# ath92/splat-renderer

Hardware: AMD Instinct MI355X
Metric: Msplats/sec (higher is better)
Workload: dtype f32

## Files before the change

### include/splat.h

```cpp
#ifndef SPLAT_H
#define SPLAT_H

#include <stddef.h>
#include <stdint.h>

#ifdef __cplusplus
extern "C" {
#endif

#define SPLAT_ABI_VERSION 3

#define SPLAT_OK 0
#define SPLAT_ERR_INVALID (-1)
#define SPLAT_ERR_HIP (-2)
#define SPLAT_ERR_OOM (-3)
#define SPLAT_ERR_CAPACITY (-4)
#define SPLAT_ERR_STATE (-5)
#define SPLAT_ERR_NO_DEVICE (-6)
#define SPLAT_ERR_COMM (-7)
#define SPLAT_ERR_RETRY (-8)

typedef struct splat_ctx splat_ctx;
typedef struct splat_sorter splat_sorter;
typedef struct splat_binner splat_binner;
// ... 46 lines not shown
                  uint32_t pr_stride_vec4, uint32_t n, void *projected, void *keys, void *payload,
                  uint32_t n_padded);

int splat_extract_keys(splat_ctx *ctx, const void *projected, uint32_t n, uint32_t n_padded,
                       void *keys, void *payload);

int splat_sort_create(splat_ctx *ctx, uint32_t capacity, splat_sorter **out);
void splat_sort_destroy(splat_sorter *s);
uint32_t splat_sort_capacity(const splat_sorter *s);
void *splat_sort_keys(splat_sorter *s);
void *splat_sort_payload(splat_sorter *s);
int splat_sort_run(splat_sorter *s, uint32_t n, uint32_t bit_begin, uint32_t bit_end);
void *splat_sort_sorted_payload(splat_sorter *s);
void *splat_sort_sorted_keys(splat_sorter *s);
int splat_probe_lds_atomic_order(splat_ctx *ctx, uint64_t *mismatches);
int splat_sort_set_mode(splat_sorter *s, int mode);
int splat_rank_status(splat_ctx *ctx, int *policy, int *atomics_ordered, uint32_t *order_faults);
#ifdef SPLAT_TEST_HOOKS
int splat_debug_inject_order_fault(splat_ctx *ctx, uint32_t tile, uint32_t position);
int splat_debug_set_tile_order(splat_ctx *ctx, const void *order_dptr);
int splat_debug_set_tile_sort_order(splat_ctx *ctx, const void *order_dptr);
int splat_debug_rerun_tile_sort(splat_ctx *ctx, splat_binner *binner);
int splat_debug_tile_sort_launches(splat_ctx *ctx, uint32_t *launches);
int splat_debug_lds_rate(splat_ctx *ctx, int kind, uint32_t workgroups_per_cu, uint32_t iters, float *ms);
#endif
int splat_composite_forget_history(splat_ctx *ctx);
int splat_composite_options(splat_ctx *ctx, int kernel, int ahead, int predict);

int splat_scan_u32(splat_ctx *ctx, const void *in, void *out, uint32_t n, void *total_dptr);

int splat_bin_create(splat_ctx *ctx, uint32_t tile_size, splat_binner **out);
void splat_bin_destroy(splat_binner *b);
int splat_bin_run(splat_binner *b, const void *projected, uint32_t n_splats, const void *sorted,
                  uint32_t n_sorted, uint32_t width, uint32_t height, uint32_t tile_row0,
                  uint32_t tile_row1);
uint32_t splat_bin_tile_size(const splat_binner *b);
int splat_bin_counts(splat_binner *b, void **dptr);
int splat_bin_offsets(splat_binner *b, void **dptr);
int splat_bin_indices(splat_binner *b, void **dptr);
int splat_bin_total(splat_binner *b, uint64_t *total_pairs);
#define SPLAT_FRAME_ORDER_DEFAULT (-1)
#define SPLAT_FRAME_SORT_FIRST 0
#define SPLAT_FRAME_TILE_FIRST 1
int splat_bin_set_frame_order(splat_binner *b, int order);
int splat_bin_dims(splat_binner *b, uint32_t *ntx, uint32_t *nty);

// ... 229 lines not shown
```

### splat_renderer_amd/_lib.py

```python
import ctypes as C
import os

_HERE = os.path.dirname(os.path.abspath(__file__))
LIB_PATH = os.environ.get("SPLAT_LIB_PATH") or os.path.join(_HERE, "libsplat_hip.so")

OK = 0
ERR_NAMES = {-1: "INVALID", -2: "HIP", -3: "OOM", -4: "CAPACITY", -5: "STATE", -6: "NO_DEVICE", -7: "COMM", -8: "RETRY"}
ERR_CAPACITY, ERR_RETRY = -4, -8
RENDER_AGAIN = (ERR_CAPACITY, ERR_RETRY)

STAGE_PROJECT, STAGE_SORT, STAGE_BIN, STAGE_COMPOSITE, STAGE_EXCHANGE, STAGE_BIN_SCATTER, STAGE_BIN_PASS2, STAGE_BIN_TILE_SORT = range(8)
STAGE_NAMES = ("project", "sort", "bin", "composite", "exchange", "bin_scatter", "bin_second_pass", "bin_tile_sort")
TIMING_COUNT_ENTRIES = 0x80000000
MODE_FRONT_TO_BACK, MODE_REFERENCE_LITERAL = 0, 1
RECORDS_PROJECTED, RECORDS_COMPACT, RECORDS_DISC48, RECORDS_LIT32 = 0, 1, 2, 3
FOOTPRINT_ISOTROPIC, FOOTPRINT_DISC, FOOTPRINT_ELLIPSOID = 0, 1, 2
U32_MAX = 0xFFFFFFFF


class SplatError(RuntimeError):
    def __init__(self, code, msg):
        super().__init__(f"libsplat_hip error {ERR_NAMES.get(code, code)}: {msg}")
        self.code = code

# ... 140 lines not shown
    "splat_band_keys": (_i, [_vp, _vp, _vp, _u32, _u32, _u32, _u32, _u32, _u32, C.POINTER(_u32)]),
    "splat_sdf_gradients": (_i, [_vp, _vp, _u32, _vp, _u32, _vp]),
    "splat_sdf_update_positions": (_i, [_vp, _vp, _vp, _u32, _vp]),
    "splat_sdf_scale_factors": (_i, [_vp, _vp, _u32, _vp, _u32, _vp]),
    "splat_sdf_curvature": (_i, [_vp, _vp, _vp, _u32, _vp]),
    "splat_sdf_seed_positions": (_i, [_vp, C.POINTER(C.c_float), C.POINTER(C.c_float), _u32, C.c_uint64, _vp]),
    "splat_sdf_generate": (_i, [_vp, _vp, _u32, C.POINTER(C.c_float), C.POINTER(C.c_float), C.c_uint64, _vp, _u32, _u32, _vp, _vp, _vp, _vp]),
    "splat_point_frame": (_i, [_vp, _vp, C.POINTER(C.c_float), _vp, _u32, _vp, _u32, _vp, _u32, _u32, _u32, _u32, _vp, _vp, _vp, _vp]),
    "splat_comm_unique_id": (_i, [_vp]),
    "splat_comm_init": (_i, [_vp, _i, _i, _vp, _pvp]),
    "splat_comm_destroy": (None, [_vp]),
    "splat_comm_rank": (_i, [_vp, C.POINTER(_i), C.POINTER(_i)]),
    "splat_comm_count": (_i, [_vp, C.POINTER(_i), C.POINTER(_i)]),
    "splat_allgather_records": (_i, [_vp, _vp, _vp, _vp, _sz]),
}
COMM_ID_BYTES = 128
HOOK_SIGNATURES = {
    "splat_debug_inject_order_fault": (_i, [_vp, _u32, _u32]),
    "splat_debug_set_tile_order": (_i, [_vp, _vp]),
    "splat_debug_set_tile_sort_order": (_i, [_vp, _vp]),
    "splat_debug_rerun_tile_sort": (_i, [_vp, _vp]),
    "splat_debug_tile_sort_launches": (_i, [_vp, C.POINTER(_u32)]),
    "splat_debug_lds_rate": (_i, [_vp, _i, _u32, _u32, C.POINTER(C.c_float)]),
}
HOOKS_LIB_PATH = os.path.join(_HERE, "libsplat_hip_hooks.so")

_lib = None


class _Bound:

    def __getattr__(self, name):
        if name in HOOK_SIGNATURES:
            raise AttributeError(f"libsplat_hip: {name} is a test hook: the shipped library does not carry it; run with "
                                 f"SPLAT_LIB_PATH={HOOKS_LIB_PATH} (the -DSPLAT_TEST_HOOKS build)")
        raise AttributeError(f"libsplat_hip: {name} is not declared in splat_renderer_amd._lib.SIGNATURES")


def load():
    global _lib
    if _lib is not None:
        return _lib
    if not os.path.exists(LIB_PATH):
        raise ImportError(
            f"{LIB_PATH} not found: build it with `python -c 'import __graft_entry__ as g; g.build()'` "
            "(hipcc --offload-arch=gfx950). splat_renderer_amd has no CPU fallback.")
# ... 25 lines not shown
```

### splat_renderer_amd/csrc/common.h

```cpp
#pragma once

#include <hip/hip_runtime.h>
#include <stdint.h>
#include <string>

#include "../../include/splat.h"

constexpr int kWave = 64;

#include <vector>
struct StageTimer {
    std::vector<hipEvent_t> beg, end;
    size_t used = 0;
    uint32_t tick = 0;
};
struct PxHistory {
    uint64_t key = 0;
    uint32_t *mem = nullptr;
    uint32_t cap = 0, parity = 0, streak = 0;
    uint64_t last_use = 0;
};
constexpr int PX_HISTORIES = 4;

struct splat_ctx {
    int device = 0;
    hipStream_t stream = nullptr;
    bool own_stream = false;
    std::string err;
    bool timing = false;
    int lds_atomic_ordered = -1;
    int rank_policy = 0;
    uint32_t order_faults = 0;
#ifdef SPLAT_TEST_HOOKS
    const uint32_t *debug_tile_order = nullptr;
    const uint32_t *debug_sort_order = nullptr;
    uint32_t inject_order_fault = 0;
    uint32_t inject_order_position = 0;
    uint32_t tile_sort_launches = 0;
#endif
    int opt_composite_kernel = -1, opt_px_ahead = 0, opt_px_predict = -1;
    PxHistory px_hist[PX_HISTORIES];
    uint64_t px_clock = 0;
    uint32_t timing_mask = 0xffffffffu;
    uint32_t timing_every = 1;
    StageTimer timers[SPLAT_STAGE_COUNT];
    void *scan_ws = nullptr;
    size_t scan_ws_bytes = 0;
    unsigned long long *d_consumed = nullptr;
    uint32_t consumed_tiles = 0;
    uint2 *d_window_counts = nullptr;
    uint32_t window_counts_cap = 0;
    void *pinned = nullptr;
    size_t pinned_bytes = 0;
};

int ctx_fail(splat_ctx *ctx, int code, const char *what, hipError_t e = hipSuccess);
bool composite_uses_px(const splat_ctx *ctx, uint32_t ntx, uint32_t nty);

int ctx_ensure_scan_ws(splat_ctx *ctx, size_t bytes);
int ctx_ensure_pinned(splat_ctx *ctx, size_t bytes);
int ctx_ensure_consumed(splat_ctx *ctx, uint32_t tiles);
// ... 193 lines not shown
```

### splat_renderer_amd/csrc/context.hip

```cpp
#include "common.h"

#include <cstdio>
#include <cstring>

static thread_local std::string g_tls_err = "";

int ctx_fail(splat_ctx *ctx, int code, const char *what, hipError_t e) {
    char buf[512];
    if (e != hipSuccess)
        snprintf(buf, sizeof buf, "%s: %s (%d)", what, hipGetErrorString(e), (int)e);
    else
        snprintf(buf, sizeof buf, "%s", what);
    if (ctx) ctx->err = buf;
    g_tls_err = buf;
    return code;
}

int ctx_ensure_scan_ws(splat_ctx *ctx, size_t bytes) {
    if (ctx->scan_ws_bytes >= bytes) return SPLAT_OK;
    if (ctx->scan_ws) {
        HIP_TRY(ctx, hipStreamSynchronize(ctx->stream));
        HIP_TRY(ctx, hipFree(ctx->scan_ws));
        ctx->scan_ws = nullptr;
        ctx->scan_ws_bytes = 0;
// ... 55 lines not shown
    (void)hipEventRecord(t.end[t.used], ctx->stream);
    ++t.used;
}

static int ctx_create_impl(int device, void *stream, bool have_stream, splat_ctx **out) {
    if (!out) return ctx_fail(nullptr, SPLAT_ERR_INVALID, "splat_ctx_create: out is NULL");
    *out = nullptr;
    int count = 0;
    hipError_t e = hipGetDeviceCount(&count);
    if (e != hipSuccess || count <= 0)
        return ctx_fail(nullptr, SPLAT_ERR_NO_DEVICE, "no HIP device visible (this library has no CPU fallback)", e);
    if (device < 0 || device >= count) return ctx_fail(nullptr, SPLAT_ERR_INVALID, "device ordinal out of range");
    e = hipSetDevice(device);
    if (e != hipSuccess) return ctx_fail(nullptr, SPLAT_ERR_HIP, "hipSetDevice", e);
    hipDeviceProp_t prop;
    e = hipGetDeviceProperties(&prop, device);
    if (e != hipSuccess) return ctx_fail(nullptr, SPLAT_ERR_HIP, "hipGetDeviceProperties", e);
    if (strncmp(prop.gcnArchName, "gfx950", 6) != 0) {
        std::string m = std::string("device is ") + prop.gcnArchName + "; libsplat_hip is built for gfx950 (MI355X) only";
        return ctx_fail(nullptr, SPLAT_ERR_NO_DEVICE, m.c_str());
    }
    splat_ctx *ctx = new splat_ctx();
    ctx->device = device;
    if (have_stream) {
        ctx->stream = (hipStream_t)stream;
        ctx->own_stream = false;
    } else {
        e = hipStreamCreateWithFlags(&ctx->stream, hipStreamNonBlocking);
        if (e != hipSuccess) {
            delete ctx;
            return ctx_fail(nullptr, SPLAT_ERR_HIP, "hipStreamCreate", e);
        }
        ctx->own_stream = true;
    }
    *out = ctx;
    return SPLAT_OK;
}

extern "C" {

int splat_abi_version(void) { return SPLAT_ABI_VERSION; }

int splat_ctx_create(int device_ordinal, splat_ctx **out) { return ctx_create_impl(device_ordinal, nullptr, false, out); }

int splat_ctx_create_on_stream(int device_ordinal, void *hip_stream, splat_ctx **out) {
    return ctx_create_impl(device_ordinal, hip_stream, true, out);
// ... 171 lines not shown
```

### splat_renderer_amd/csrc/frame.hip

```cpp
#include "common.h"
#include "tile_range.h"
#include "disc.h"
#include "ellipsoid.h"
#include "shade.h"

#include <cstdlib>

__device__ __forceinline__ uint32_t depth_key_of(float depth) {
    uint32_t bits = __float_as_uint(depth);
    uint32_t mask = ((bits >> 31) == 1u) ? 0xffffffffu : 0x80000000u;
    return bits ^ mask;
}

__global__ __launch_bounds__(256) void k_band_flag(const float4 *__restrict__ projected, uint32_t n, uint32_t width,
                                                   uint32_t height, uint32_t tile, uint32_t ntx, uint32_t nty, uint32_t row0,
                                                   uint32_t row1, uint32_t *__restrict__ flags) {
    uint32_t i = blockIdx.x * 256u + threadIdx.x;
    if (i >= n) return;
    uint32_t a, b, c, d;
    flags[i] = tile_range(projected[(size_t)i * 2], width, height, tile, ntx, nty, row0, row1, a, b, c, d) ? 1u : 0u;
}

__global__ __launch_bounds__(256) void k_band_scatter(const float4 *__restrict__ projected, uint32_t n,
                                                      const uint32_t *__restrict__ slot, const uint32_t *__restrict__ total,
// ... 645 lines not shown
                                                "in all)");
    int rc = SPLAT_OK;
    uint32_t *range32 = nullptr;
    uint2 *range_wide = nullptr;
    const BinParams bp = {width, height, tile, ntx, nty, row0, row1, (row0 > 0 || row1 < nty) ? 1u : 0u};
    if (ell && bp.skip_outside)
        return ctx_fail(ctx, SPLAT_ERR_INVALID, "splat_render_frame_ellipsoids: the ellipsoid footprint has no band frame (render every tile row)");
    if (fast) {
        rc = binner_reserve_range32(binner, n);
        if (rc != SPLAT_OK) return rc;
        range32 = binner->range32;
    } else if (wide) {
        rc = binner_reserve_range_wide(binner, n);
        if (rc != SPLAT_OK) return rc;
        range_wide = reinterpret_cast<uint2 *>(binner->range32);
    }
    ARG_CHECK(ctx, (((uintptr_t)props | (uintptr_t)projected) & 15) == 0);
    const bool tile_first = fast && frame_order(binner) == SPLAT_FRAME_TILE_FIRST;
    TfHistOut ho = {};
    const bool band_compact = tile_first && bp.skip_outside && band_compacting(row0, row1, nty);
    if (tile_first) {
        rc = binner_reserve(binner, ntx * nty, n);
        if (rc != SPLAT_OK) return rc;
        const uint32_t block = band_compact ? BTC_GROUP : (n <= TF_SMALL_FRAME_SPLATS && !bp.skip_outside) ? TF_BLOCK_SMALL : TF_BLOCK_LARGE;
        ho = {binner->tf_hist, binner->blocksums, binner->d_total + 1, (1u << tile_id_low_bits(ntx * nty)) - 1u, div_up(n, block), block};
        binner->tf_block = block;
        if (band_compact) {
            rc = binner_reserve_band_idx(ctx, binner, n);
            if (rc != SPLAT_OK) return rc;
            ho.cidx = binner->band_idx;
            ho.kept_groups = sorter->hist;
        }
    }
    if (disc && n > binner->discs_cap) {
        HIP_TRY(ctx, hipStreamSynchronize(ctx->stream));
        if (binner->discs) (void)hipFree(binner->discs);
        binner->discs = nullptr;
        binner->discs_cap = 0;
        if (hipMalloc(&binner->discs, (size_t)n * 48 + 256) != hipSuccess) return ctx_fail(ctx, SPLAT_ERR_OOM, "disc records hipMalloc");
        binner->discs_cap = n;
    }
    if (ctx->timing) {
        rc = ctx_ensure_consumed(ctx, ntx * nty);
        if (rc != SPLAT_OK) return rc;
    }
    const LitIO lio = {(const float4 *)color, (const float4 *)normals, color_stride, 1u, cfg->prelit,
                       lit ? (float4 *)projected : disc_lit ? (float4 *)binner->discs : nullptr};
// ... 87 lines not shown
```

### splat_renderer_amd/csrc/radix_sort.hip

```cpp
#include "common.h"

#include <cstdlib>

constexpr uint32_t RS_THREADS = 256;
constexpr uint32_t RS_ITEMS = RADIX_PART / RS_THREADS;
constexpr uint32_t RS_WAVES = RS_THREADS / 64;

constexpr uint32_t RS_PART_KEYS = RS_ITEMS * RS_THREADS;

__device__ __forceinline__ uint32_t sort_count(uint32_t n_host, const uint32_t *n_dev) {
    if (!n_dev) return n_host;
    const uint32_t v = *n_dev;
    return v < n_host ? v : n_host;
}

__device__ __forceinline__ void hist_add4(uint32_t *h, uint4 v, uint32_t shift, uint32_t mask) {
    const uint32_t a = (v.x >> shift) & mask, b = (v.y >> shift) & mask, c = (v.z >> shift) & mask, d = (v.w >> shift) & mask;
    if (a == b && b == c && c == d) {
        atomicAdd(&h[a], 4u);
    } else {
        atomicAdd(&h[a], 1u);
        atomicAdd(&h[b], 1u);
        atomicAdd(&h[c], 1u);
        atomicAdd(&h[d], 1u);
// ... 580 lines not shown
    if (!ctx) return ctx_fail(nullptr, SPLAT_ERR_INVALID, "ctx is NULL");
    ctx->debug_sort_order = (const uint32_t *)order_dptr;
    return SPLAT_OK;
}

int splat_debug_set_tile_order(splat_ctx *ctx, const void *order_dptr) {
    if (!ctx) return ctx_fail(nullptr, SPLAT_ERR_INVALID, "ctx is NULL");
    ctx->debug_tile_order = (const uint32_t *)order_dptr;
    return SPLAT_OK;
}

int splat_debug_lds_rate(splat_ctx *ctx, int kind, uint32_t workgroups_per_cu, uint32_t iters, float *ms) {
    if (!ctx || !ms) return ctx_fail(ctx, SPLAT_ERR_INVALID, "ctx/ms is NULL");
    ARG_CHECK(ctx, kind >= 0 && kind <= 2 && workgroups_per_cu >= 1 && workgroups_per_cu <= 8 && iters >= 1 && iters <= (1u << 20));
    return radix_probe_lds_rate(ctx, kind, workgroups_per_cu, iters, ms);
}

int splat_debug_tile_sort_launches(splat_ctx *ctx, uint32_t *launches) {
    if (!ctx || !launches) return ctx_fail(nullptr, SPLAT_ERR_INVALID, "ctx/launches is NULL");
    *launches = ctx->tile_sort_launches;
    return SPLAT_OK;
}

int splat_debug_inject_order_fault(splat_ctx *ctx, uint32_t tile, uint32_t position) {
    if (!ctx) return ctx_fail(nullptr, SPLAT_ERR_INVALID, "ctx is NULL");
    ARG_CHECK(ctx, tile != 0xffffffffu);
    ARG_CHECK(ctx, position < 0x3fffffffu);
    ctx->inject_order_fault = tile + 1u;
    ctx->inject_order_position = position;
    return SPLAT_OK;
}
#endif

int splat_probe_lds_atomic_order(splat_ctx *ctx, uint64_t *mismatches) {
    if (!ctx || !mismatches) return ctx_fail(nullptr, SPLAT_ERR_INVALID, "ctx/mismatches is NULL");
    return radix_probe_lds_atomic_order(ctx, mismatches);
}

void *splat_sort_sorted_keys(splat_sorter *s) {
    if (!s) return nullptr;
    return s->result_in_primary ? s->keys : s->keys_b;
}

}
```

### splat_renderer_amd/csrc/tile_first.hip

```cpp
#include "common.h"
#include "tile_range.h"

constexpr uint32_t TF_THREADS = 256;
constexpr uint32_t TF_STAGE = 4096;
static_assert(TF_BLOCK_LARGE == 1024 && TF_BLOCK_SMALL == 256, "the stage word packs the block-local slot in 10 bits; blocks are 256 x {4, 1}");

__device__ __forceinline__ uint32_t range32_hits(uint32_t r) {
    const uint32_t tx0 = r & 0xffu, tx1 = (r >> 8) & 0xffu, ty0 = (r >> 16) & 0xffu, ty1 = r >> 24;
    return (tx0 > tx1 || ty0 > ty1) ? 0u : (tx1 - tx0 + 1) * (ty1 - ty0 + 1);
}

constexpr uint32_t TS_THREADS = 256, TS_WAVES = 4;
constexpr uint32_t TS_LONG_ITEMS = 24;
constexpr uint32_t TS_LDS_ELEMS = 5888;
constexpr uint32_t TS_CHUNK_ITEMS = 16;

struct TileSortShared {
    uint32_t wave_hist[TS_WAVES][256];
    uint32_t digit_base[256];
    uint32_t wave_sums[TS_WAVES];
    uint32_t kmin, kmax;
};

template <bool RANK_ATOMIC>
// ... 32 lines not shown
        const uint32_t t = __shfl_up(incl, s);
        if ((int)lane >= s) incl += t;
    }
    if (lane == 63) wave_sums[w] = incl;
    __syncthreads();
    const uint32_t wprefix = (w > 0 ? wave_sums[0] : 0u) + (w > 1 ? wave_sums[1] : 0u) + (w > 2 ? wave_sums[2] : 0u);
    __syncthreads();
    return wprefix + incl - v;
}

constexpr uint32_t TFS_ITEMS = TF_STAGE / TF_THREADS;

struct TfScatterShared {
    uint32_t wave_hist[TS_WAVES][256];
    uint32_t digit_base[256];
    uint32_t global_base[256];
    uint32_t wave_sums[TS_WAVES];
};

#ifndef TF_SCATTER_WAVES
#define TF_SCATTER_WAVES 5
#endif
constexpr uint32_t TF_GROUP = 4096;
template <bool RANK_ATOMIC, uint32_t TF_PER_THREAD, bool COMPACTED = false>
__global__ __launch_bounds__(TF_THREADS, TF_SCATTER_WAVES) void k_tf_scatter(const uint32_t *__restrict__ range32,
                                                           const uint32_t *__restrict__ depth_keys, uint32_t n, uint32_t ntx,
                                                           uint32_t mask, uint32_t num_parts,
                                                           const uint32_t *__restrict__ scanned_hist,
                                                           const uint32_t *__restrict__ totals, uint32_t *__restrict__ d_total,
                                                           uint32_t pair_limit, uint32_t *__restrict__ overflow,
                                                           uint8_t *__restrict__ out_hi, uint2 *__restrict__ out_val,
                                                           uint32_t lo_bits, uint32_t align_m1, TfRuns runs,
                                                           uint32_t *__restrict__ offsets_out, uint32_t tiles, uint32_t *report,
                                                           uint32_t seq, const uint32_t *__restrict__ cidx,
                                                           const uint32_t *__restrict__ kept, uint32_t xcd_per) {
    static_assert(!COMPACTED || TF_PER_THREAD == 4, "compacted groups are read four splats per thread");
    const uint32_t blk = xcd_block_of(blockIdx.x, xcd_per);
    if (blk >= num_parts) return;
    __shared__ TfScatterShared sh;
    __shared__ uint32_t wsum[4];
    __shared__ uint32_t stage[TF_STAGE];
    __shared__ uint32_t s_key[TF_THREADS * TF_PER_THREAD];
    __shared__ uint32_t s_idx[COMPACTED ? TF_THREADS * TF_PER_THREAD : 1];
    const uint32_t tid = threadIdx.x, lane = tid & 63, w = tid >> 6;
    uint32_t first = blk * (COMPACTED ? TF_GROUP : TF_THREADS * TF_PER_THREAD);
    if (COMPACTED) n = first + min(kept[blk], TF_GROUP);
    static_assert(TF_PER_THREAD == 4 || TF_PER_THREAD == 1, "uint4 or scalar loads");
    uint32_t i0 = first + tid * TF_PER_THREAD;
    uint4 rr = make_uint4(1u, 1u, 1u, 1u), kk = make_uint4(0, 0, 0, 0);
    if (TF_PER_THREAD == 1) {
        if (i0 < n) { rr.x = range32[i0]; kk.x = depth_keys[i0]; }
    } else if (i0 + 3 < n) {
        rr = reinterpret_cast<const uint4 *>(range32)[i0 >> 2];
        kk = reinterpret_cast<const uint4 *>(depth_keys)[i0 >> 2];
    } else {
        if (i0 < n) { rr.x = range32[i0]; kk.x = depth_keys[i0]; }
        if (i0 + 1 < n) { rr.y = range32[i0 + 1]; kk.y = depth_keys[i0 + 1]; }
        if (i0 + 2 < n) { rr.z = range32[i0 + 2]; kk.z = depth_keys[i0 + 2]; }
    }
    const uint32_t digit_total = totals[tid];
    const uint32_t row_prefix = tid <= mask ? scanned_hist[(size_t)tid * num_parts + blk] : 0u;

    const uint32_t digit_room = (digit_total + align_m1) & ~align_m1;
    uint32_t gincl = digit_total, aincl = digit_room;
    unsigned long long g64 = digit_total;
#pragma unroll
    for (int s = 1; s < 64; s <<= 1) {
        const uint32_t t = __shfl_up(gincl, s), a = __shfl_up(aincl, s);
        const unsigned long long t64 = __shfl_up(g64, s);
        if ((int)lane >= s) {
            gincl += t;
            aincl += a;
            g64 += t64;
        }
    }
    __shared__ unsigned long long wsum64[4];
    if (lane == 63) {
        sh.wave_sums[w] = gincl;
        wsum[w] = aincl;
        wsum64[w] = g64;
    }
    __syncthreads();
    const uint32_t aprefix = (w > 0 ? wsum[0] : 0u) + (w > 1 ? wsum[1] : 0u) + (w > 2 ? wsum[2] : 0u);
    const unsigned long long all_pairs64 = wsum64[0] + wsum64[1] + wsum64[2] + wsum64[3];
// ... 2 lines not shown
    if (blk == 0) {
        const bool fits = all_pairs <= pair_limit;
        if (tid == 0) {
            d_total[0] = all_pairs;
            d_total[2] = fits ? all_pairs : 0u;
            d_total[3] = 0u;
            if (!fits) atomicOr(overflow, 1u);
        }
        runs.start[tid] = fits ? run_start : 0u;
        runs.total[tid] = fits ? digit_total : 0u;
        if (align_m1 && fits)
            for (uint32_t j = 0, first_part = run_start / (align_m1 + 1u); j < digit_room / (align_m1 + 1u); ++j)
                runs.part_digit[first_part + j] = (uint8_t)tid;
        if (tid == 255) *runs.parts = (align_m1 && fits) ? (run_start + digit_room) / (align_m1 + 1u) : 0u;
        if (offsets_out) {
            if (tid < tiles) offsets_out[tid] = fits ? run_start : 0u;
            if (tid == 0) {
                offsets_out[tiles] = fits ? all_pairs : 0u;
                if (report) tile_report(d_total, report, seq);
            }
        }
    }
    if (all_pairs > pair_limit) return;
    sh.global_base[tid] = run_start + row_prefix;
    for (;;) {
    __syncthreads();

    uint32_t r[TF_PER_THREAD], h[TF_PER_THREAD];
    if constexpr (TF_PER_THREAD == 4) {
        reinterpret_cast<uint4 *>(s_key)[tid] = kk;
        r[0] = rr.x; r[1] = rr.y; r[2] = rr.z; r[3] = rr.w;
        if constexpr (COMPACTED) {
            uint4 ii = make_uint4(0, 0, 0, 0);
            if (i0 + 3 < n) ii = reinterpret_cast<const uint4 *>(cidx)[i0 >> 2];
            else {
                if (i0 < n) ii.x = cidx[i0];
                if (i0 + 1 < n) ii.y = cidx[i0 + 1];
                if (i0 + 2 < n) ii.z = cidx[i0 + 2];
            }
            reinterpret_cast<uint4 *>(s_idx)[tid] = ii;
        }
    } else {
        s_key[tid] = kk.x;
        r[0] = rr.x;
    }
#pragma unroll
    for (uint32_t k = 0; k < TF_PER_THREAD; ++k) h[k] = range32_hits(r[k]);
    uint32_t off[TF_PER_THREAD];
    uint32_t carry;
    {
        uint32_t mine = 0;
#pragma unroll
        for (uint32_t k = 0; k < TF_PER_THREAD; ++k) mine += h[k];
        uint32_t incl = mine;
#pragma unroll
        for (int d = 1; d < 64; d <<= 1) {
            const uint32_t t = __shfl_up(incl, d);
            if ((int)lane >= d) incl += t;
        }
        if (lane == 63) wsum[w] = incl;
        __syncthreads();
        const uint32_t s0 = wsum[0], s1 = wsum[1], s2 = wsum[2], s3 = wsum[3];
        off[0] = (w > 0 ? s0 : 0u) + (w > 1 ? s1 : 0u) + (w > 2 ? s2 : 0u) + incl - mine;
#pragma unroll
        for (uint32_t k = 1; k < TF_PER_THREAD; ++k) off[k] = off[k - 1] + h[k - 1];
        carry = s0 + s1 + s2 + s3;
    }
    const uint32_t total = carry;
    const bool more_splats = COMPACTED && first + TF_THREADS * TF_PER_THREAD < n;
    if (total == 0 && !more_splats) return;
    for (uint32_t c0 = 0; c0 < total; c0 += TF_STAGE) {
        const uint32_t cnt = (total - c0 < TF_STAGE) ? total - c0 : TF_STAGE;
        for (uint32_t i = tid; i < TS_WAVES * 256; i += TF_THREADS) (&sh.wave_hist[0][0])[i] = 0;
#pragma unroll
        for (uint32_t k = 0; k < TF_PER_THREAD; ++k) {
            if (h[k] == 0 || off[k] >= c0 + TF_STAGE || off[k] + h[k] <= c0) continue;
            const uint32_t tx0 = r[k] & 0xffu, tx1 = (r[k] >> 8) & 0xffu, ty0 = (r[k] >> 16) & 0xffu, ty1 = r[k] >> 24;
            const uint32_t slot = tid * TF_PER_THREAD + k;
            uint32_t o = off[k] - c0;
            for (uint32_t ty = ty0; ty <= ty1; ++ty)
                for (uint32_t tx = tx0; tx <= tx1; ++tx) {
                    if (o < TF_STAGE) stage[o] = ((ty * ntx + tx) << 10) | slot;
                    ++o;
                }
        }
        __syncthreads();
        const uint32_t items = ((cnt + TF_THREADS - 1) / TF_THREADS + 3u) & ~3u;
        const uint32_t wbase = w * items * 64 + lane;
        uint32_t el[TFS_ITEMS], rank[TFS_ITEMS];
#pragma unroll
        for (uint32_t g = 0; g < TFS_ITEMS; g += 4) {
            if (g < items) {
#pragma unroll
                for (uint32_t i = g; i < g + 4; ++i) {
                    const uint32_t p = wbase + i * 64;
                    el[i] = stage[p < cnt ? p : cnt - 1];
                }
#pragma unroll
                for (uint32_t i = g; i < g + 4; ++i) {
                    rank[i] = 0;
                    if (wbase + i * 64 < cnt) rank[i] = wave_rank<RANK_ATOMIC>(sh.wave_hist[w], (el[i] >> 10) & mask);
                }
            }
        }
        __syncthreads();
        const uint32_t dcount = ts_wave_prefixes(sh.wave_hist, tid);
        const uint32_t excl = ts_scan256(sh.wave_sums, dcount, tid);
        sh.digit_base[tid] = excl;
        __syncthreads();
#pragma unroll
        for (uint32_t g = 0; g < TFS_ITEMS; g += 4) {
            if (g < items) {
#pragma unroll
                for (uint32_t i = g; i < g + 4; ++i) {
                    const uint32_t d = (el[i] >> 10) & mask;
                    if (wbase + i * 64 < cnt) stage[sh.digit_base[d] + sh.wave_hist[w][d] + rank[i]] = el[i];
                }
            }
        }
        __syncthreads();
        for (uint32_t pos = tid; pos < cnt; pos += TF_THREADS) {
            const uint32_t e = stage[pos], slot = e & 1023u, d = (e >> 10) & mask;
            const uint32_t g = sh.global_base[d] + (pos - sh.digit_base[d]);
            out_hi[g] = (uint8_t)(e >> (10u + lo_bits));
            out_val[g] = make_uint2(s_key[slot], COMPACTED ? s_idx[slot] : first + slot);
        }
        if (c0 + TF_STAGE >= total && !more_splats) break;
        __syncthreads();
        sh.global_base[tid] += dcount;
        __syncthreads();
    }
    if (!more_splats) return;
    first += TF_THREADS * TF_PER_THREAD;
    {
        const uint32_t j0 = first + tid * TF_PER_THREAD;
        rr = make_uint4(1u, 1u, 1u, 1u);
        kk = make_uint4(0, 0, 0, 0);
        if (j0 + 3 < n) {
            rr = reinterpret_cast<const uint4 *>(range32)[j0 >> 2];
            kk = reinterpret_cast<const uint4 *>(depth_keys)[j0 >> 2];
        } else {
            if (j0 < n) { rr.x = range32[j0]; kk.x = depth_keys[j0]; }
            if (j0 + 1 < n) { rr.y = range32[j0 + 1]; kk.y = depth_keys[j0 + 1]; }
            if (j0 + 2 < n) { rr.z = range32[j0 + 2]; kk.z = depth_keys[j0 + 2]; }
        }
        i0 = j0;
    }
    }
}

__device__ __forceinline__ void tile_list_out(uint2 *s_el, uint32_t n, uint32_t *__restrict__ out, uint32_t *frame_flags, bool inject,
                                              uint32_t inject_pos, uint32_t tid) {
    const uint32_t lane = tid & 63, w = tid >> 6;
    if (inject) {
        if (tid == 0 && n >= inject_pos + 2u) {
            const uint2 a = s_el[inject_pos];
            s_el[inject_pos] = s_el[inject_pos + 1];
            s_el[inject_pos + 1] = a;
        }
        __syncthreads();
    }
    bool bad = false;
    for (uint32_t s0 = 0; s0 * 63u < n; s0 += 4 * TS_WAVES) {
        uint2 a[4];
#pragma unroll
        for (uint32_t i = 0; i < 4; ++i) {
            const uint32_t p = (s0 + i * TS_WAVES + w) * 63u + lane;
            a[i] = s_el[p < n ? p : n - 1];
        }
#pragma unroll
// ... 467 lines not shown
        int rc = radix_rowscan_launch(ctx, hist, num_parts, hmask + 1u);
        if (rc != SPLAT_OK) return rc;
        const TfOffsetsArgs off = {tiles, lo_bits, offsets, d_total};
        const dim3 grid(part_blocks + div_up(tiles + 1, 256));
        const bool ra = rank_atomic_ok(ctx, true);
        const uint32_t pad = hi_bits >= 8u ? 4096u : 0u;
        if (ra)
            hipLaunchKernelGGL((k_tf_downsweep2<true, 4>), grid, dim3(TF_THREADS), pad, ctx->stream, hi, val_in, val_out, *runs, hmask, num_parts, hist,
                               totals, off, part_blocks, xcd_per);
        else
            hipLaunchKernelGGL((k_tf_downsweep2<false, 4>), grid, dim3(TF_THREADS), pad, ctx->stream, hi, val_in, val_out, *runs, hmask, num_parts, hist,
                               totals, off, part_blocks, xcd_per);
        LAUNCH_CHECK(ctx, "k_tf_downsweep2");
    }
    return SPLAT_OK;
}

int tf_scatter_launch(splat_ctx *ctx, const uint32_t *range32, const uint32_t *depth_keys, uint32_t n, uint32_t ntx, uint32_t mask,
                      const uint32_t *hist, uint32_t *d_total, uint32_t pair_limit, uint32_t *overflow, uint8_t *out_hi,
                      uint2 *out_val, uint32_t block_splats, uint32_t lo_bits, bool second_pass, const TfRuns *runs,
                      uint32_t *offsets_if_final, uint32_t tiles, uint32_t *report, uint32_t seq, const uint32_t *cidx,
                      const uint32_t *kept) {
    const uint32_t parts = div_up(n, block_splats);
    const uint32_t xcd_per = parts >= 64u ? div_up(parts, 8u) : 0u;
    const uint32_t grid_blocks = xcd_per ? 8u * xcd_per : parts;
    if (cidx && block_splats != TF_GROUP) return ctx_fail(ctx, SPLAT_ERR_INVALID, "tf_scatter_launch: compacted input comes in groups of 4096 records");
    const uint32_t *totals = hist + (size_t)256 * parts;
    {
        int prc = ctx_resolve_rank_mode(ctx);
        if (prc != SPLAT_OK) return prc;
    }
    const bool ra = rank_atomic_ok(ctx, true);
#define SPLAT_TF_SCATTER_(RA, PER, COMPACTED)                                                                                     \
    hipLaunchKernelGGL((k_tf_scatter<RA, PER, COMPACTED>), dim3(grid_blocks), dim3(TF_THREADS), 0, ctx->stream, range32, depth_keys, n, ntx, mask, parts, \
                       hist, totals, d_total, pair_limit, overflow, out_hi, out_val, lo_bits, second_pass ? TF_RUN_ALIGN - 1u : 0u, *runs,         \
                       second_pass ? nullptr : offsets_if_final, tiles, report, seq, cidx, kept, xcd_per)
#define SPLAT_TF_SCATTER(RA, PER) SPLAT_TF_SCATTER_(RA, PER, false)
    if (cidx) {
        if (ra) SPLAT_TF_SCATTER_(true, 4, true);
        else SPLAT_TF_SCATTER_(false, 4, true);
    } else if (block_splats == TF_BLOCK_SMALL) {
        if (ra) SPLAT_TF_SCATTER(true, 1);
        else SPLAT_TF_SCATTER(false, 1);
    } else {
        if (ra) SPLAT_TF_SCATTER(true, 4);
        else SPLAT_TF_SCATTER(false, 4);
    }
#undef SPLAT_TF_SCATTER
// ... 5 lines not shown
```

### splat_renderer_amd/host.py

```python
import ctypes as C

import numpy as np

from . import _lib
from ._lib import CompositeCfg, SplatError, check

U32_MAX = 0xFFFFFFFF


class Buffer:

    def __init__(self, device, ptr, size, owned=True):
        self.device, self.ptr, self.size, self._owned = device, ptr, int(size), owned
        self._host_shadow = None

    def destroy(self):
        if self._owned and self.ptr:
            check(self.device.lib.splat_buf_free(self.device.ctx, self.ptr), self.device.ctx)
        self.ptr = None

    def write(self, array, offset=0):
        a = np.ascontiguousarray(array)
        if offset + a.nbytes > self.size:
            raise ValueError("write past the end of the buffer")
# ... 74 lines not shown
    def setTiming(self, enabled=True):
        check(self.lib.splat_set_timing(self.ctx, int(enabled)), self.ctx)

    def stageTimeMs(self, stage):
        ms = C.c_float()
        check(self.lib.splat_stage_time_ms(self.ctx, stage, C.byref(ms)), self.ctx)
        return float(ms.value)

    def rankStatus(self):
        pol, ordered, faults = C.c_int(), C.c_int(), C.c_uint32()
        check(self.lib.splat_rank_status(self.ctx, C.byref(pol), C.byref(ordered), C.byref(faults)), self.ctx)
        return {"policy": ("checked", "atomic", "ballot")[pol.value], "atomicsOrdered": bool(ordered.value == 1),
                "orderFaults": int(faults.value)}

    def forgetCompositeHistory(self):
        check(self.lib.splat_composite_forget_history(self.ctx), self.ctx)

    def compositeOptions(self, kernel=None, ahead=0, predict=None):
        k = -1 if kernel is None else {"quadrant": 0, "pixel": 1}[kernel]
        check(self.lib.splat_composite_options(self.ctx, k, int(ahead), -1 if predict is None else int(bool(predict))), self.ctx)

    def injectOrderFault(self, tile, position=0):
        check(self.lib.splat_debug_inject_order_fault(self.ctx, int(tile), int(position)), self.ctx)

    def tileSortLaunches(self):
        v = C.c_uint32(0)
        check(self.lib.splat_debug_tile_sort_launches(self.ctx, C.byref(v)), self.ctx)
        return int(v.value)

    def destroy(self):
        if self.ctx:
            self.lib.splat_ctx_destroy(self.ctx)
            self.ctx = None


def _uniform_floats(u):
    if isinstance(u, Buffer):
        if u._host_shadow is None:
            raise SplatError(-1, "uniform buffer was never written")
        u = u._host_shadow.view(np.float32)
    u = np.ascontiguousarray(u, dtype=np.float32)
    return u


class PointManager:

# ... 849 lines not shown
```

Measured before the change: 15650.

## Make tile scatter persistent with prefetched double-buffered next block

For the large-block non-compacted tile scatter path, the grid is capped at the number of resident workgroups (waves per CU times CU count), and each workgroup loops over several blocks. While it ranks and writes the current block, it prefetches the next block's ranges, keys and histogram prefix into registers and a second LDS key buffer. The aim is to hide global load latency and cut launch and tail overhead for large frames. The cost is more LDS and register pressure and considerably more complex control flow, plus a test hook to override residency.

```diff
diff --git a/include/splat.h b/include/splat.h
--- a/include/splat.h
+++ b/include/splat.h
@@ -92,6 +92,7 @@
 int splat_debug_set_tile_sort_order(splat_ctx *ctx, const void *order_dptr);
 int splat_debug_rerun_tile_sort(splat_ctx *ctx, splat_binner *binner);
 int splat_debug_tile_sort_launches(splat_ctx *ctx, uint32_t *launches);
+int splat_debug_set_binning_residency(splat_ctx *ctx, uint32_t workgroups);
 int splat_debug_lds_rate(splat_ctx *ctx, int kind, uint32_t workgroups_per_cu, uint32_t iters, float *ms);
 #endif
 int splat_composite_forget_history(splat_ctx *ctx);
diff --git a/splat_renderer_amd/_lib.py b/splat_renderer_amd/_lib.py
--- a/splat_renderer_amd/_lib.py
+++ b/splat_renderer_amd/_lib.py
@@ -186,6 +186,7 @@
     "splat_debug_rerun_tile_sort": (_i, [_vp, _vp]),
     "splat_debug_tile_sort_launches": (_i, [_vp, C.POINTER(_u32)]),
     "splat_debug_lds_rate": (_i, [_vp, _i, _u32, _u32, C.POINTER(C.c_float)]),
+    "splat_debug_set_binning_residency": (_i, [_vp, _u32]),
 }
 HOOKS_LIB_PATH = os.path.join(_HERE, "libsplat_hip_hooks.so")
 
diff --git a/splat_renderer_amd/csrc/common.h b/splat_renderer_amd/csrc/common.h
--- a/splat_renderer_amd/csrc/common.h
+++ b/splat_renderer_amd/csrc/common.h
@@ -24,6 +24,7 @@
 
 struct splat_ctx {
     int device = 0;
+    uint32_t cu_count = 0;
     hipStream_t stream = nullptr;
     bool own_stream = false;
     std::string err;
@@ -37,6 +38,7 @@
     uint32_t inject_order_fault = 0;
     uint32_t inject_order_position = 0;
     uint32_t tile_sort_launches = 0;
+    uint32_t debug_binning_residency = 0;
 #endif
     int opt_composite_kernel = -1, opt_px_ahead = 0, opt_px_predict = -1;
     PxHistory px_hist[PX_HISTORIES];
diff --git a/splat_renderer_amd/csrc/context.hip b/splat_renderer_amd/csrc/context.hip
--- a/splat_renderer_amd/csrc/context.hip
+++ b/splat_renderer_amd/csrc/context.hip
@@ -101,6 +101,7 @@
     }
     splat_ctx *ctx = new splat_ctx();
     ctx->device = device;
+    ctx->cu_count = prop.multiProcessorCount > 0 ? (uint32_t)prop.multiProcessorCount : 1u;
     if (have_stream) {
         ctx->stream = (hipStream_t)stream;
         ctx->own_stream = false;
diff --git a/splat_renderer_amd/csrc/frame.hip b/splat_renderer_amd/csrc/frame.hip
--- a/splat_renderer_amd/csrc/frame.hip
+++ b/splat_renderer_amd/csrc/frame.hip
@@ -691,7 +691,11 @@
     if (tile_first) {
         rc = binner_reserve(binner, ntx * nty, n);
         if (rc != SPLAT_OK) return rc;
-        const uint32_t block = band_compact ? BTC_GROUP : (n <= TF_SMALL_FRAME_SPLATS && !bp.skip_outside) ? TF_BLOCK_SMALL : TF_BLOCK_LARGE;
+        bool small_blocks = n <= TF_SMALL_FRAME_SPLATS && !bp.skip_outside;
+#ifdef SPLAT_TEST_HOOKS
+        if (ctx->debug_binning_residency) small_blocks = false;
+#endif
+        const uint32_t block = band_compact ? BTC_GROUP : small_blocks ? TF_BLOCK_SMALL : TF_BLOCK_LARGE;
         ho = {binner->tf_hist, binner->blocksums, binner->d_total + 1, (1u << tile_id_low_bits(ntx * nty)) - 1u, div_up(n, block), block};
         binner->tf_block = block;
         if (band_compact) {
diff --git a/splat_renderer_amd/csrc/radix_sort.hip b/splat_renderer_amd/csrc/radix_sort.hip
--- a/splat_renderer_amd/csrc/radix_sort.hip
+++ b/splat_renderer_amd/csrc/radix_sort.hip
@@ -626,6 +626,12 @@
     return SPLAT_OK;
 }
 
+int splat_debug_set_binning_residency(splat_ctx *ctx, uint32_t workgroups) {
+    if (!ctx) return ctx_fail(nullptr, SPLAT_ERR_INVALID, "ctx is NULL");
+    ctx->debug_binning_residency = workgroups;
+    return SPLAT_OK;
+}
+
 int splat_debug_inject_order_fault(splat_ctx *ctx, uint32_t tile, uint32_t position) {
     if (!ctx) return ctx_fail(nullptr, SPLAT_ERR_INVALID, "ctx is NULL");
     ARG_CHECK(ctx, tile != 0xffffffffu);
diff --git a/splat_renderer_amd/csrc/tile_first.hip b/splat_renderer_amd/csrc/tile_first.hip
--- a/splat_renderer_amd/csrc/tile_first.hip
+++ b/splat_renderer_amd/csrc/tile_first.hip
@@ -78,6 +78,42 @@
 #define TF_SCATTER_WAVES 5
 #endif
 constexpr uint32_t TF_GROUP = 4096;
+__device__ __forceinline__ uint32_t tf_here(uint32_t v) {
+    asm volatile("" : "+v"(v));
+    return v;
+}
+template <uint32_t TF_PER_THREAD>
+__device__ __forceinline__ void tf_load_block(const uint32_t *__restrict__ range32, const uint32_t *__restrict__ depth_keys, uint32_t first,
+                                              uint32_t tid, uint32_t n, uint4 &rr, uint4 &kk) {
+    static_assert(TF_PER_THREAD == 4 || TF_PER_THREAD == 1, "uint4 or scalar loads");
+    tid = tf_here(tid);
+    const uint32_t *r = range32 + first, *k = depth_keys + first;
+    const uint32_t t0 = tid * TF_PER_THREAD, i0 = first + t0;
+    rr = make_uint4(1u, 1u, 1u, 1u);
+    kk = make_uint4(0, 0, 0, 0);
+    if (TF_PER_THREAD == 1) {
+        if (i0 < n) { rr.x = r[t0]; kk.x = k[t0]; }
+    } else if (i0 + 3 < n) {
+        rr = reinterpret_cast<const uint4 *>(r)[tid];
+        kk = reinterpret_cast<const uint4 *>(k)[tid];
+    } else {
+        if (i0 < n) { rr.x = r[t0]; kk.x = k[t0]; }
+        if (i0 + 1 < n) { rr.y = r[t0 + 1]; kk.y = k[t0 + 1]; }
+        if (i0 + 2 < n) { rr.z = r[t0 + 2]; kk.z = k[t0 + 2]; }
+    }
+}
+typedef uint32_t tf_u32x4 __attribute__((ext_vector_type(4)));
+__device__ __forceinline__ void tf_arrived(tf_u32x4 &v) { asm volatile("" : "+v"(v)); }
+__device__ __forceinline__ void tf_arrived(uint4 &v) {
+    tf_u32x4 t = {v.x, v.y, v.z, v.w};
+    asm volatile("" : "+v"(t));
+    v = make_uint4(t.x, t.y, t.z, t.w);
+}
+__device__ __forceinline__ uint32_t tf_hist_entry(const uint32_t *__restrict__ scanned_hist, uint32_t num_parts, uint32_t digit, uint32_t blk) {
+    uint32_t offset = digit * num_parts * 4u;
+    asm volatile("" : "+v"(offset));
+    return *reinterpret_cast<const uint32_t *>(reinterpret_cast<const char *>(scanned_hist + blk) + offset);
+}
 template <bool RANK_ATOMIC, uint32_t TF_PER_THREAD, bool COMPACTED = false>
 __global__ __launch_bounds__(TF_THREADS, TF_SCATTER_WAVES) void k_tf_scatter(const uint32_t *__restrict__ range32,
                                                            const uint32_t *__restrict__ depth_keys, uint32_t n, uint32_t ntx,
@@ -91,31 +127,28 @@
                                                            uint32_t seq, const uint32_t *__restrict__ cidx,
                                                            const uint32_t *__restrict__ kept, uint32_t xcd_per) {
     static_assert(!COMPACTED || TF_PER_THREAD == 4, "compacted groups are read four splats per thread");
-    const uint32_t blk = xcd_block_of(blockIdx.x, xcd_per);
-    if (blk >= num_parts) return;
+    constexpr bool RESIDENT = !COMPACTED && TF_PER_THREAD == 4;
+    constexpr uint32_t BLOCK_SPLATS = TF_THREADS * TF_PER_THREAD;
+    const uint32_t xcd_base = xcd_per ? (blockIdx.x & 7u) * xcd_per : 0u, local_end = xcd_per ? xcd_per : num_parts;
+    const uint32_t local_stride = xcd_per ? gridDim.x >> 3 : gridDim.x;
+    uint32_t local = xcd_per ? blockIdx.x >> 3 : blockIdx.x;
+    uint32_t blk = xcd_base + local;
+    if (local >= local_end || blk >= num_parts) return;
     __shared__ TfScatterShared sh;
     __shared__ uint32_t wsum[4];
     __shared__ uint32_t stage[TF_STAGE];
-    __shared__ uint32_t s_key[TF_THREADS * TF_PER_THREAD];
-    __shared__ uint32_t s_idx[COMPACTED ? TF_THREADS * TF_PER_THREAD : 1];
+    __shared__ uint32_t s_key_mem[BLOCK_SPLATS * (RESIDENT ? 2 : 1)];
+    __shared__ uint32_t s_idx[COMPACTED ? BLOCK_SPLATS : 1];
+    __shared__ uint32_t s_prefix_next[RESIDENT ? TF_THREADS : 1];
+    uint32_t *s_key = s_key_mem;
     const uint32_t tid = threadIdx.x, lane = tid & 63, w = tid >> 6;
-    uint32_t first = blk * (COMPACTED ? TF_GROUP : TF_THREADS * TF_PER_THREAD);
+    uint32_t first = blk * (COMPACTED ? TF_GROUP : BLOCK_SPLATS);
     if (COMPACTED) n = first + min(kept[blk], TF_GROUP);
-    static_assert(TF_PER_THREAD == 4 || TF_PER_THREAD == 1, "uint4 or scalar loads");
     uint32_t i0 = first + tid * TF_PER_THREAD;
-    uint4 rr = make_uint4(1u, 1u, 1u, 1u), kk = make_uint4(0, 0, 0, 0);
-    if (TF_PER_THREAD == 1) {
-        if (i0 < n) { rr.x = range32[i0]; kk.x = depth_keys[i0]; }
-    } else if (i0 + 3 < n) {
-        rr = reinterpret_cast<const uint4 *>(range32)[i0 >> 2];
-        kk = reinterpret_cast<const uint4 *>(depth_keys)[i0 >> 2];
-    } else {
-        if (i0 < n) { rr.x = range32[i0]; kk.x = depth_keys[i0]; }
-        if (i0 + 1 < n) { rr.y = range32[i0 + 1]; kk.y = depth_keys[i0 + 1]; }
-        if (i0 + 2 < n) { rr.z = range32[i0 + 2]; kk.z = depth_keys[i0 + 2]; }
-    }
+    uint4 rr, kk;
+    tf_load_block<TF_PER_THREAD>(range32, depth_keys, first, tid, n, rr, kk);
     const uint32_t digit_total = totals[tid];
-    const uint32_t row_prefix = tid <= mask ? scanned_hist[(size_t)tid * num_parts + blk] : 0u;
+    uint32_t row_prefix = tid <= mask ? tf_hist_entry(scanned_hist, num_parts, tid, blk) : 0u;
 
     const uint32_t digit_room = (digit_total + align_m1) & ~align_m1;
     uint32_t gincl = digit_total, aincl = digit_room;
@@ -164,13 +197,54 @@
         }
     }
     if (all_pairs > pair_limit) return;
-    sh.global_base[tid] = run_start + row_prefix;
+    if constexpr (RESIDENT) {
+        reinterpret_cast<uint4 *>(s_key)[tid] = kk;
+        asm volatile("" : "+v"(row_prefix));
+        tf_arrived(rr);
+    } else {
+        sh.global_base[tid] = run_start + row_prefix;
+    }
+    uint32_t c0 = 0, dcount = 0;
+    bool has_next = false, next_whole = false, parked = true;
     for (;;) {
     __syncthreads();
+    tf_u32x4 rr_n = {1u, 1u, 1u, 1u}, kk_n = {0u, 0u, 0u, 0u};
+    uint32_t row_prefix_n = 0;
+    if constexpr (RESIDENT) {
+        if (c0 == 0) {
+            sh.global_base[tid] = run_start + row_prefix;
+            local += local_stride;
+            has_next = local < local_end && xcd_base + local < num_parts;
+            next_whole = has_next && (xcd_base + local + 1u) * BLOCK_SPLATS <= n;
+            parked = !next_whole;
+        } else {
+            sh.global_base[tid] += dcount;
+        }
+        if (next_whole) {
+            const uint32_t nblk = xcd_base + local, t = tf_here(tid);
+            rr_n = reinterpret_cast<const tf_u32x4 *>(range32 + nblk * BLOCK_SPLATS)[t];
+            if (!parked) {
+                kk_n = reinterpret_cast<const tf_u32x4 *>(depth_keys + nblk * BLOCK_SPLATS)[t];
+                row_prefix_n = tid <= mask ? tf_hist_entry(scanned_hist, num_parts, tid, nblk) : 0u;
+            }
+        }
+    }
+    auto tf_next_arrived = [&]() __attribute__((always_inline)) {
+        if constexpr (RESIDENT) {
+            asm volatile("" : "+v"(row_prefix_n));
+            tf_arrived(rr_n);
+            tf_arrived(kk_n);
+            if (!parked) {
+                reinterpret_cast<tf_u32x4 *>(s_key == s_key_mem ? s_key_mem + BLOCK_SPLATS : s_key_mem)[tid] = kk_n;
+                s_prefix_next[tid] = row_prefix_n;
+                parked = true;
+            }
+        }
+    };
 
     uint32_t r[TF_PER_THREAD], h[TF_PER_THREAD];
     if constexpr (TF_PER_THREAD == 4) {
-        reinterpret_cast<uint4 *>(s_key)[tid] = kk;
+        if constexpr (!RESIDENT) reinterpret_cast<uint4 *>(s_key)[tid] = kk;
         r[0] = rr.x; r[1] = rr.y; r[2] = rr.z; r[3] = rr.w;
         if constexpr (COMPACTED) {
             uint4 ii = make_uint4(0, 0, 0, 0);
@@ -188,8 +262,7 @@
     }
 #pragma unroll
     for (uint32_t k = 0; k < TF_PER_THREAD; ++k) h[k] = range32_hits(r[k]);
-    uint32_t off[TF_PER_THREAD];
-    uint32_t carry;
+    uint32_t off0, carry;
     {
         uint32_t mine = 0;
 #pragma unroll
@@ -203,23 +276,26 @@
         if (lane == 63) wsum[w] = incl;
         __syncthreads();
         const uint32_t s0 = wsum[0], s1 = wsum[1], s2 = wsum[2], s3 = wsum[3];
-        off[0] = (w > 0 ? s0 : 0u) + (w > 1 ? s1 : 0u) + (w > 2 ? s2 : 0u) + incl - mine;
-#pragma unroll
-        for (uint32_t k = 1; k < TF_PER_THREAD; ++k) off[k] = off[k - 1] + h[k - 1];
+        off0 = (w > 0 ? s0 : 0u) + (w > 1 ? s1 : 0u) + (w > 2 ? s2 : 0u) + incl - mine;
         carry = s0 + s1 + s2 + s3;
     }
     const uint32_t total = carry;
-    const bool more_splats = COMPACTED && first + TF_THREADS * TF_PER_THREAD < n;
-    if (total == 0 && !more_splats) return;
-    for (uint32_t c0 = 0; c0 < total; c0 += TF_STAGE) {
+    const bool more_splats = COMPACTED && first + BLOCK_SPLATS < n;
+    if constexpr (!RESIDENT)
+        if (total == 0 && !more_splats) return;
+    auto tf_round = [&](const uint32_t c0) __attribute__((always_inline)) -> uint32_t {
         const uint32_t cnt = (total - c0 < TF_STAGE) ? total - c0 : TF_STAGE;
         for (uint32_t i = tid; i < TS_WAVES * 256; i += TF_THREADS) (&sh.wave_hist[0][0])[i] = 0;
+        uint32_t off_k = off0;
 #pragma unroll
         for (uint32_t k = 0; k < TF_PER_THREAD; ++k) {
-            if (h[k] == 0 || off[k] >= c0 + TF_STAGE || off[k] + h[k] <= c0) continue;
+            if constexpr (TF_PER_THREAD > 1) asm volatile("" : "+v"(r[k]));
+            const uint32_t h_k = range32_hits(r[k]), o_k = off_k;
+            off_k += h_k;
+            if (h_k == 0 || o_k >= c0 + TF_STAGE || o_k + h_k <= c0) continue;
             const uint32_t tx0 = r[k] & 0xffu, tx1 = (r[k] >> 8) & 0xffu, ty0 = (r[k] >> 16) & 0xffu, ty1 = r[k] >> 24;
             const uint32_t slot = tid * TF_PER_THREAD + k;
-            uint32_t o = off[k] - c0;
+            uint32_t o = o_k - c0;
             for (uint32_t ty = ty0; ty <= ty1; ++ty)
                 for (uint32_t tx = tx0; tx <= tx1; ++tx) {
                     if (o < TF_STAGE) stage[o] = ((ty * ntx + tx) << 10) | slot;
@@ -227,9 +303,10 @@
                 }
         }
         __syncthreads();
+        tf_next_arrived();
         const uint32_t items = ((cnt + TF_THREADS - 1) / TF_THREADS + 3u) & ~3u;
         const uint32_t wbase = w * items * 64 + lane;
-        uint32_t el[TFS_ITEMS], rank[TFS_ITEMS];
+        uint32_t el[TFS_ITEMS], rank2[TFS_ITEMS / 2];
 #pragma unroll
         for (uint32_t g = 0; g < TFS_ITEMS; g += 4) {
             if (g < items) {
@@ -240,8 +317,9 @@
                 }
 #pragma unroll
                 for (uint32_t i = g; i < g + 4; ++i) {
-                    rank[i] = 0;
-                    if (wbase + i * 64 < cnt) rank[i] = wave_rank<RANK_ATOMIC>(sh.wave_hist[w], (el[i] >> 10) & mask);
+                    uint32_t rk = 0;
+                    if (wbase + i * 64 < cnt) rk = wave_rank<RANK_ATOMIC>(sh.wave_hist[w], (el[i] >> 10) & mask);
+                    rank2[i >> 1] = (i & 1u) ? rank2[i >> 1] | (rk << 16) : rk;
                 }
             }
         }
@@ -256,7 +334,8 @@
 #pragma unroll
                 for (uint32_t i = g; i < g + 4; ++i) {
                     const uint32_t d = (el[i] >> 10) & mask;
-                    if (wbase + i * 64 < cnt) stage[sh.digit_base[d] + sh.wave_hist[w][d] + rank[i]] = el[i];
+                    const uint32_t rk = (i & 1u) ? rank2[i >> 1] >> 16 : rank2[i >> 1] & 0xffffu;
+                    if (wbase + i * 64 < cnt) stage[sh.digit_base[d] + sh.wave_hist[w][d] + rk] = el[i];
                 }
             }
         }
@@ -267,27 +346,45 @@
             out_hi[g] = (uint8_t)(e >> (10u + lo_bits));
             out_val[g] = make_uint2(s_key[slot], COMPACTED ? s_idx[slot] : first + slot);
         }
-        if (c0 + TF_STAGE >= total && !more_splats) break;
-        __syncthreads();
-        sh.global_base[tid] += dcount;
+        return dcount;
+    };
+    if constexpr (RESIDENT) {
+        dcount = tf_round(c0);
+        c0 += TF_STAGE;
+        if (c0 < total) {
+            uint4 kk_again;
+            tf_load_block<TF_PER_THREAD>(range32, depth_keys, first, tid, n, rr, kk_again);
+            tf_arrived(rr);
+            continue;
+        }
+        c0 = 0;
+        if (!has_next) return;
+        blk = xcd_base + local;
+        first = blk * BLOCK_SPLATS;
+        if (first + BLOCK_SPLATS > n) {
+            uint4 rr_last, kk_last;
+            tf_load_block<TF_PER_THREAD>(range32, depth_keys, first, tid, n, rr_last, kk_last);
+            s_prefix_next[tid] = tid <= mask ? tf_hist_entry(scanned_hist, num_parts, tid, blk) : 0u;
+            reinterpret_cast<uint4 *>(s_key == s_key_mem ? s_key_mem + BLOCK_SPLATS : s_key_mem)[tid] = kk_last;
+            rr_n = tf_u32x4{rr_last.x, rr_last.y, rr_last.z, rr_last.w};
+            tf_arrived(rr_n);
+        }
+        rr = make_uint4(rr_n.x, rr_n.y, rr_n.z, rr_n.w);
+        row_prefix = s_prefix_next[tid];
+        s_key = s_key == s_key_mem ? s_key_mem + BLOCK_SPLATS : s_key_mem;
+        continue;
+    }
+    for (uint32_t c1 = 0; c1 < total; c1 += TF_STAGE) {
+        const uint32_t dcount1 = tf_round(c1);
+        if (c1 + TF_STAGE >= total && !more_splats) break;
+        __syncthreads();
+        sh.global_base[tid] += dcount1;
         __syncthreads();
     }
     if (!more_splats) return;
-    first += TF_THREADS * TF_PER_THREAD;
-    {
-        const uint32_t j0 = first + tid * TF_PER_THREAD;
-        rr = make_uint4(1u, 1u, 1u, 1u);
-        kk = make_uint4(0, 0, 0, 0);
-        if (j0 + 3 < n) {
-            rr = reinterpret_cast<const uint4 *>(range32)[j0 >> 2];
-            kk = reinterpret_cast<const uint4 *>(depth_keys)[j0 >> 2];
-        } else {
-            if (j0 < n) { rr.x = range32[j0]; kk.x = depth_keys[j0]; }
-            if (j0 + 1 < n) { rr.y = range32[j0 + 1]; kk.y = depth_keys[j0 + 1]; }
-            if (j0 + 2 < n) { rr.z = range32[j0 + 2]; kk.z = depth_keys[j0 + 2]; }
-        }
-        i0 = j0;
-    }
+    first += BLOCK_SPLATS;
+    i0 = first + tid * TF_PER_THREAD;
+    tf_load_block<TF_PER_THREAD>(range32, depth_keys, first, tid, n, rr, kk);
     }
 }
 
@@ -801,8 +898,18 @@
                       uint32_t *offsets_if_final, uint32_t tiles, uint32_t *report, uint32_t seq, const uint32_t *cidx,
                       const uint32_t *kept) {
     const uint32_t parts = div_up(n, block_splats);
-    const uint32_t xcd_per = parts >= 64u ? div_up(parts, 8u) : 0u;
-    const uint32_t grid_blocks = xcd_per ? 8u * xcd_per : parts;
+    uint32_t xcd_per = parts >= 64u ? div_up(parts, 8u) : 0u;
+    uint32_t grid_blocks = xcd_per ? 8u * xcd_per : parts;
+    if (!cidx && block_splats == TF_BLOCK_LARGE) {
+        uint32_t resident = (uint32_t)TF_SCATTER_WAVES * ctx->cu_count;
+#ifdef SPLAT_TEST_HOOKS
+        if (ctx->debug_binning_residency) resident = ctx->debug_binning_residency;
+#endif
+        if (resident < grid_blocks) {
+            if (resident < 8u) xcd_per = 0u;
+            grid_blocks = xcd_per ? resident & ~7u : resident;
+        }
+    }
     if (cidx && block_splats != TF_GROUP) return ctx_fail(ctx, SPLAT_ERR_INVALID, "tf_scatter_launch: compacted input comes in groups of 4096 records");
     const uint32_t *totals = hist + (size_t)256 * parts;
     {
diff --git a/splat_renderer_amd/host.py b/splat_renderer_amd/host.py
--- a/splat_renderer_amd/host.py
+++ b/splat_renderer_amd/host.py
@@ -120,6 +120,9 @@
 
     def injectOrderFault(self, tile, position=0):
         check(self.lib.splat_debug_inject_order_fault(self.ctx, int(tile), int(position)), self.ctx)
+
+    def setBinningResidency(self, workgroups=0):
+        check(self.lib.splat_debug_set_binning_residency(self.ctx, int(workgroups)), self.ctx)
 
     def tileSortLaunches(self):
         v = C.c_uint32(0)
```

After: 15750 (median of 5 runs). No clear change (+0.7%).
